# PNP-team/ZPrize23-gpu-submission

Hardware: AMD Instinct MI355X
Metric: gen_proof wall-clock (s), HEIGHT=15 Poseidon tree, 1/2/4/8 MI355X + HBM GB/s (lower is better)
Workload: dtype u64

## Files before the change

### zprize23-gpu-submission_amd/csrc/fr29.cuh

```cuda
#pragma once
#include "field.cuh"
#include "fr29_consts.inc"

namespace pnp {

struct R29 {
    uint32_t l[9];
};

#define R29_M 0x1FFFFFFFu

__device__ __forceinline__ R29 r29_from_words(const uint32_t *v) {
    R29 r;
#pragma unroll
    for (int j = 0; j < 9; j++) {
        const int bit = 29 * j, w = bit >> 5, sh = bit & 31;
        uint32_t x = v[w] >> sh;
        if (sh > 3 && w + 1 < 8) x |= v[w + 1] << (32 - sh);
        r.l[j] = j < 8 ? (x & R29_M) : x;
    }
    return r;
}

__device__ __forceinline__ void r29_to_words(const R29 &a, uint32_t *v) {
// ... 60 lines not shown
    R29 r;
    uint64_t acc = 0;
#pragma unroll
    for (int k = 0; k < 17; k++) {
#pragma unroll
        for (int i = (k > 8 ? k - 8 : 0); i <= (k < 8 ? k : 8); i++) {
            acc += (uint64_t)a.l[i] * b.l[k - i];
            acc += (uint64_t)c.l[i] * d.l[k - i];
        }
#pragma unroll
        for (int i = (k > 8 ? k - 8 : 0); i < (k < 9 ? k : 9); i++) acc += (uint64_t)m[i] * R29_P[k - i];
        if (k < 9) {
            m[k] = (0u - (uint32_t)acc) & R29_M;
            acc += m[k];
        } else {
            r.l[k - 9] = (uint32_t)acc & R29_M;
        }
        acc >>= 29;
    }
    r.l[8] = (uint32_t)acc;
    return r;
}

__device__ __forceinline__ R29 r29_canon(const R29 &x) {
    const uint32_t q = (uint32_t)(((uint64_t)x.l[8] * R29_MU) >> 32);
    R29 y;
    uint64_t acc = 0;
#pragma unroll
    for (int i = 0; i < 8; i++) {
        acc += x.l[i] + (uint64_t)q * R29_C[i];
        y.l[i] = (uint32_t)acc & R29_M;
        acc >>= 29;
    }
    y.l[8] = (uint32_t)(acc + x.l[8] + (uint64_t)q * R29_C[8] - ((uint64_t)q << 29));
#pragma unroll
    for (int rep = 0; rep < 2; rep++) {
        R29 z;
        uint32_t c = 0;
#pragma unroll
        for (int i = 0; i < 8; i++) {
            const uint32_t t = y.l[i] + R29_C[i] + c;
            z.l[i] = t & R29_M;
            c = t >> 29;
        }
        const uint32_t t = y.l[8] + R29_C[8] + c;
        const bool ge = t >= (1u << 29);
// ... 17 lines not shown
```

### zprize23-gpu-submission_amd/csrc/protocol.h

```cpp
#pragma once
#include "pnp_internal.h"

namespace pnp {

__host__ __device__ inline Fr from_u64_limbs_dev(const uint64_t *l) {
    Fr r;
#pragma unroll
    for (int i = 0; i < 4; i++) {
        r.v[2 * i] = (uint32_t)l[i];
        r.v[2 * i + 1] = (uint32_t)(l[i] >> 32);
    }
    return r;
}

struct PermArgs {
    const uint64_t *w[4];
    const uint64_t *sigma[4];
    Fr bk[4];
    Fr beta, gamma, omega;
    const uint64_t *tw;
};

struct QuotArgs {
    const uint64_t *w8[4], *z8, *pi8, *f8, *t8, *h18, *h28, *z28, *l18;
    const uint64_t *q_m, *q_l, *q_r, *q_o, *q_4, *q_c, *q_hl, *q_hr, *q_h4, *q_arith, *q_lookup;
    const uint64_t *sig[4], *lin, *vh_inv;
    const uint64_t *l1v, *pinv;
    Fr c_pi;
    uint64_t n;
    uint32_t lg_n;
    Fr alpha, alpha2, beta, gamma, delta, eps, zeta, lsep;
    Fr bk[4], opd, eopd, sep2, sep3;
};

struct Quot29Args {
    const uint64_t *w8[4], *z8, *pi8;
    const uint64_t *q_m, *q_l, *q_r, *q_o, *q_4, *q_c, *q_hl, *q_hr, *q_h4, *q_arith;
    const uint64_t *sig[4], *lin;
    const uint64_t *vh_inv, *l1v, *pinv;
    uint32_t c_pi[9], alpha[9], alpha2[9], beta[9], gamma[9], one[9];
    uint64_t n;
    uint32_t lg_n;
};
void fr_to_r29_limbs(const Fr &a, uint32_t l[9]);
void k_quotient29(const Quot29Args &q, uint64_t N8, uint64_t *out, hipStream_t s);
void k_to_form29(const uint64_t *in, uint64_t *out, uint64_t n, hipStream_t s);

struct WidgetArgs {
    const uint64_t *w8[4], *q_l, *q_r, *q_c, *vh_inv;
    const uint64_t *sel[4];
    Fr sep[4];
    uint64_t n;
    uint32_t lg_n;
};

constexpr int LIN_MAX = 32;
struct LinArgs {
    int k;
    const uint64_t *p[LIN_MAX];
    Fr s[LIN_MAX];
};

void k_compress4(uint64_t *out, const uint64_t *t0, const uint64_t *t1, const uint64_t *t2,
                 const uint64_t *t3, const Fr &z, uint64_t n, hipStream_t s);
void k_query_f(uint64_t *out, const uint64_t *ql, uint64_t n_gates, const uint64_t *const w[4],
               const uint64_t *tc, const Fr &z, uint64_t n, hipStream_t s);
void k_perm_numden(uint64_t *num, uint64_t *den, const PermArgs &a, uint64_t n, hipStream_t s);
void k_lookup_nd(uint64_t *num, uint64_t *den, const uint64_t *f, const uint64_t *t,
                 const uint64_t *h1, const uint64_t *h2, const Fr &delta, const Fr &eps, uint64_t n,
                 hipStream_t s);
void k_mul_inplace(uint64_t *a, const uint64_t *b, uint64_t n, hipStream_t s);
bool k_any_nonzero(const uint64_t *v, uint64_t words, DevBuf &scratch, hipStream_t s);
void k_any_nonzero_n(const uint64_t *v, uint64_t words, uint64_t stride, int cnt, bool *nz, DevBuf &scratch,
                     hipStream_t s);
bool k_any_diff(const uint64_t *a, const uint64_t *b, uint64_t words, DevBuf &scratch, hipStream_t s);
void k_hash_words(const uint64_t *a, uint64_t words, DevBuf &scratch, hipStream_t s, uint64_t out[2]);
bool k_pack_affine(const uint8_t *src, uint64_t n, uint64_t stride, uint64_t x_off, uint64_t y_off,
                   uint64_t inf_off, uint64_t *dst, DevBuf &scratch, hipStream_t s);
void k_affine(uint64_t *out, const uint64_t *in, const Fr &a, const Fr &b, uint64_t n, hipStream_t s);
void k_quotient(const QuotArgs &q, uint64_t N8, uint64_t *out, hipStream_t s);
void k_lincomb(const LinArgs &a, uint64_t n, uint64_t *out, hipStream_t s);
void k_widgets(const WidgetArgs &g, uint64_t N8, uint64_t *out, hipStream_t s);
bool combine_split(pnp_ctx *ctx, const uint64_t *t, const uint64_t *f, uint64_t n, uint64_t *h1,
                   uint64_t *h2, hipStream_t s);
void k_proof_marker(hipStream_t s);

}
```

### zprize23-gpu-submission_amd/csrc/protocol.hip

```cpp
#include "pnp_internal.h"
#include "protocol.h"
#include "widgets.cuh"
#include "fr29.cuh"
#include <vector>

namespace pnp {

static inline uint32_t nblk(uint64_t threads, uint32_t bs = 256) {
    return (uint32_t)((threads + bs - 1) / bs);
}

__global__ void k_compress4_(uint64_t *out, const uint64_t *t0, const uint64_t *t1,
                             const uint64_t *t2, const uint64_t *t3, Fr z, uint64_t n) {
    uint64_t i = blockIdx.x * (uint64_t)blockDim.x + threadIdx.x;
    if (i >= n) return;
    Fr acc = load_fr(t3, i);
    acc = acc * z + load_fr(t2, i);
    acc = acc * z + load_fr(t1, i);
    acc = acc * z + load_fr(t0, i);
    store_fr(out, i, acc);
}
void k_compress4(uint64_t *out, const uint64_t *t0, const uint64_t *t1, const uint64_t *t2,
                 const uint64_t *t3, const Fr &z, uint64_t n, hipStream_t s) {
    hipLaunchKernelGGL(k_compress4_, dim3(nblk(n)), dim3(256), 0, s, out, t0, t1, t2, t3, z, n);
    PNP_HIP(hipGetLastError());
}
// ... 59 lines not shown
    Fr eopd = eps * opd;
    const uint64_t nx = (i + 1) & (n - 1);
    Fr tn = load_fr(t, nx), h1n = load_fr(h1, nx);
    Fr fi = load_fr(f, i), ti = load_fr(t, i), h1i = load_fr(h1, i), h2i = load_fr(h2, i);
    Fr r = (eopd + ti + delta * tn) * (opd * (eps + fi));
    Fr d = (h2i * delta + (eopd + h1i)) * ((eopd + h2i) + h1n * delta);
    store_fr(num, i, r);
    store_fr(den, i, d);
}
void k_lookup_nd(uint64_t *num, uint64_t *den, const uint64_t *f, const uint64_t *t,
                 const uint64_t *h1, const uint64_t *h2, const Fr &delta, const Fr &eps, uint64_t n,
                 hipStream_t s) {
    hipLaunchKernelGGL(k_lookup_nd_, dim3(nblk(n)), dim3(256), 0, s, num, den, f, t, h1, h2, delta, eps,
                       n);
    PNP_HIP(hipGetLastError());
}

__global__ void k_mul_inplace_(uint64_t *a, const uint64_t *b, uint64_t n) {
    uint64_t i = blockIdx.x * (uint64_t)blockDim.x + threadIdx.x;
    if (i < n) store_fr(a, i, load_fr(a, i) * load_fr(b, i));
}
void k_mul_inplace(uint64_t *a, const uint64_t *b, uint64_t n, hipStream_t s) {
    hipLaunchKernelGGL(k_mul_inplace_, dim3(nblk(n)), dim3(256), 0, s, a, b, n);
    PNP_HIP(hipGetLastError());
}

__global__ __launch_bounds__(256) void k_any_nonzero_(const uint64_t *v, uint64_t words, uint64_t stride,
                                                      unsigned *flag) {
    const ulonglong2 *p = reinterpret_cast<const ulonglong2 *>(v + stride * blockIdx.y);
    const uint64_t pairs = words / 2;
    uint64_t acc = 0;
    for (uint64_t i = blockIdx.x * (uint64_t)blockDim.x + threadIdx.x; i < pairs;
         i += (uint64_t)gridDim.x * blockDim.x) {
        const ulonglong2 x = p[i];
        acc |= x.x | x.y;
    }
    if (blockIdx.x == 0 && threadIdx.x == 0 && (words & 1)) acc |= v[stride * blockIdx.y + words - 1];
    if (__any(acc != 0) && (threadIdx.x & 63) == 0) atomicOr(flag + blockIdx.y, 1u);
}
void k_any_nonzero_n(const uint64_t *v, uint64_t words, uint64_t stride, int cnt, bool *nz, DevBuf &scratch,
                     hipStream_t s) {
    scratch.reserve(4 * (size_t)cnt + 16);
    unsigned *flag = static_cast<unsigned *>(scratch.p);
    PNP_HIP(hipMemsetAsync(flag, 0, 4 * (size_t)cnt, s));
    if (words) {
        uint64_t blocks = (words / 2 + 255) / 256;
// ... 157 lines not shown
    }
    if (q.z28) {
        Fr tt = ld(q.t8, i), ttn = ld(q.t8, nx);
        Fr h1 = ld(q.h18, i), h1n = ld(q.h18, nx), h2 = ld(q.h28, i);
        Fr z2 = load_fr(q.z28, i), z2n = load_fr(q.z28, nx);
        Fr lk = z2 * q.opd * (f + q.eps) * (tt + q.eopd + ttn * q.delta) * q.sep2;
        lk -= z2n * (h1 + q.eopd + h2 * q.delta) * (h2 + q.eopd + h1n * q.delta) * q.sep2;
        l1t += (z2 - Fr::one()) * q.sep3;
        num += lk;
    }
    if (q.l1v) {
        Fr r = fr_mul2(num, load_fr(q.vh_inv, i), l1t, load_fr(q.l1v, i));
        if (q.pinv) r += q.c_pi * load_fr(q.pinv, i);
        store_fr(out, i, r);
    } else {
        store_fr(out, i, (num + l1t * load_fr(q.l18, i)) * load_fr(q.vh_inv, i));
    }
}
void k_quotient(const QuotArgs &q, uint64_t N8, uint64_t *out, hipStream_t s) {
    hipLaunchKernelGGL(k_quotient_, dim3(nblk(N8)), dim3(256), 0, s, q, N8, out);
    PNP_HIP(hipGetLastError());
}

__device__ __forceinline__ R29 ld29(const uint64_t *p, uint64_t i) {
    const uint4 *q = reinterpret_cast<const uint4 *>(p + 4 * i);
    const uint4 lo = q[0], hi = q[1];
    const uint32_t w[8] = {lo.x, lo.y, lo.z, lo.w, hi.x, hi.y, hi.z, hi.w};
    return r29_from_words(w);
}
__device__ __forceinline__ R29 c29(const uint32_t *c) {
    R29 r;
#pragma unroll
    for (int k = 0; k < 9; k++) r.l[k] = c[k];
    return r;
}
__device__ __forceinline__ R29 pow5_29(const R29 &a) {
    const R29 a2 = r29_mul(a, a);
    return r29_mul(r29_mul(a2, a2), a);
}
__device__ __forceinline__ R29 add3_29(const R29 &a, const R29 &b, const R29 &c) {
    return r29_add(r29_add(a, b), c);
}

__global__ __launch_bounds__(256, 4) void k_quotient29_(Quot29Args q, uint64_t N8, uint64_t *out) {
    const uint64_t i = blockIdx.x * (uint64_t)blockDim.x + threadIdx.x;
    if (i >= N8) return;
    const uint64_t nx = next_in_block(i, q.n, q.lg_n);
    const R29 a = ld29(q.w8[0], i), b = ld29(q.w8[1], i), c = ld29(q.w8[2], i), d = ld29(q.w8[3], i);
    R29 acc = r29_mul2(a, ld29(q.q_l, i), b, ld29(q.q_r, i));
    if (q.q_m) acc = r29_add(acc, r29_mul(r29_mul(a, b), ld29(q.q_m, i)));
    acc = r29_add(acc, r29_mul2(c, ld29(q.q_o, i), d, ld29(q.q_4, i)));
    acc = r29_add(acc, r29_mul2(pow5_29(a), ld29(q.q_hl, i), pow5_29(b), ld29(q.q_hr, i)));
    acc = r29_add(acc, r29_mul(pow5_29(d), ld29(q.q_h4, i)));
    acc = r29_add(acc, ld29(q.q_c, i));
    R29 num = r29_mul(acc, ld29(q.q_arith, i));
    if (q.pi8) num = r29_add(num, ld29(q.pi8, i));
    const R29 beta = c29(q.beta), gamma = c29(q.gamma);
    const R29 xb = r29_mul(ld29(q.lin, i), beta);
    const R29 x2 = r29_add(xb, xb), x4 = r29_add(x2, x2), x8 = r29_add(x4, x4);
    const R29 xb7 = r29_sub(x8, xb, R29_KDIF[0]);
    const R29 xb13 = add3_29(x8, x4, xb), xb17 = add3_29(x8, x8, xb);
    R29 pa = r29_mul(add3_29(xb, a, gamma), add3_29(xb7, b, gamma));
    pa = r29_mul(pa, add3_29(xb13, c, gamma));
    pa = r29_mul(pa, add3_29(xb17, d, gamma));
    R29 pb = r29_mul(add3_29(r29_mul(ld29(q.sig[0], i), beta), a, gamma),
                     add3_29(r29_mul(ld29(q.sig[1], i), beta), b, gamma));
    pb = r29_mul(pb, add3_29(r29_mul(ld29(q.sig[2], i), beta), c, gamma));
    pb = r29_mul(pb, add3_29(r29_mul(ld29(q.sig[3], i), beta), d, gamma));
    const R29 zi = ld29(q.z8, i), zn = ld29(q.z8, nx);
    R29 zero;
#pragma unroll
    for (int k = 0; k < 9; k++) zero.l[k] = 0;
    const R29 nzn = r29_sub(zero, zn, R29_KDIF[0]);
    num = r29_add(num, r29_mul(r29_mul2(pa, zi, pb, nzn), c29(q.alpha)));
    const R29 l1t = r29_mul(r29_sub(zi, c29(q.one), R29_KDIF[0]), c29(q.alpha2));
    R29 r = r29_mul2(num, ld29(q.vh_inv, i), l1t, ld29(q.l1v, i));
    if (q.pinv) r = r29_add(r, r29_mul(c29(q.c_pi), ld29(q.pinv, i)));
    r = r29_canon(r);
    uint32_t w[8];
    r29_to_words(r, w);
    uint4 *o = reinterpret_cast<uint4 *>(out + 4 * i);
    o[0] = make_uint4(w[0], w[1], w[2], w[3]);
    o[1] = make_uint4(w[4], w[5], w[6], w[7]);
}
void k_quotient29(const Quot29Args &q, uint64_t N8, uint64_t *out, hipStream_t s) {
    hipLaunchKernelGGL(k_quotient29_, dim3(nblk(N8)), dim3(256), 0, s, q, N8, out);
    PNP_HIP(hipGetLastError());
}

__global__ void k_to_form29_(const uint64_t *in, uint64_t *out, uint64_t n) {
    const uint64_t i = blockIdx.x * (uint64_t)blockDim.x + threadIdx.x;
    if (i >= n) return;
    Fr x = load_fr(in, i);
#pragma unroll
    for (int k = 0; k < 5; k++) x = x + x;
    store_fr(out, i, x);
}
void k_to_form29(const uint64_t *in, uint64_t *out, uint64_t n, hipStream_t s) {
    hipLaunchKernelGGL(k_to_form29_, dim3(nblk(n)), dim3(256), 0, s, in, out, n);
    PNP_HIP(hipGetLastError());
}

void fr_to_r29_limbs(const Fr &a, uint32_t l[9]) {
    Fr x = a;
    for (int k = 0; k < 5; k++) x = x + x;
    for (int j = 0; j < 9; j++) {
        const int bit = 29 * j, w = bit >> 5, sh = bit & 31;
        uint64_t v = x.v[w] >> sh;
        if (w + 1 < 8) v |= (uint64_t)x.v[w + 1] << (32 - sh);
        l[j] = j < 8 ? (uint32_t)(v & 0x1FFFFFFFu) : (uint32_t)v;
    }
}

__global__ __launch_bounds__(256) void k_widgets_(WidgetArgs g, uint64_t N8, uint64_t *out) {
    uint64_t i = blockIdx.x * (uint64_t)blockDim.x + threadIdx.x;
    if (i >= N8) return;
    const uint64_t nx = next_in_block(i, g.n, g.lg_n);
    WidgetVals w;
    w.a = load_fr(g.w8[0], i);
    w.b = load_fr(g.w8[1], i);
    w.c = load_fr(g.w8[2], i);
    w.d = load_fr(g.w8[3], i);
    w.a_next = load_fr(g.w8[0], nx);
    w.b_next = load_fr(g.w8[1], nx);
    w.d_next = load_fr(g.w8[3], nx);
    w.q_l = load_fr(g.q_l, i);
    w.q_r = load_fr(g.q_r, i);
    w.q_c = load_fr(g.q_c, i);
    Fr acc = Fr::zero();
    if (g.sel[0]) acc += load_fr(g.sel[0], i) * w_range(g.sep[0], w);
    if (g.sel[1]) acc += load_fr(g.sel[1], i) * w_logic(g.sep[1], w);
    if (g.sel[2]) acc += load_fr(g.sel[2], i) * w_fbsm(g.sep[2], w);
    if (g.sel[3]) acc += load_fr(g.sel[3], i) * w_cadd(g.sep[3], w);
    store_fr(out, i, load_fr(out, i) + acc * load_fr(g.vh_inv, i));
// ... 30 lines not shown
```

### zprize23-gpu-submission_amd/csrc/prover.cpp

```cpp
#include <chrono>
#include <string.h>
#include "context.h"
#include "protocol.h"
#include "transcript.h"
#include "widgets.cuh"
#include <algorithm>
#include <stddef.h>

namespace pnp {

Fr fr_from_u64(uint64_t x) {
    Fr r = Fr::zero();
    r.v[0] = (uint32_t)x;
    r.v[1] = (uint32_t)(x >> 32);
    return to_mont(r);
}

Fr root_of_unity(uint32_t lg) {
    const uint64_t root32[4] = {13381757501831005802ULL, 6564924994866501612ULL,
                                789602057691799140ULL, 6625830629041353339ULL};
    return pow_u64(from_u64_limbs<FrP>(root32), 1ULL << (32 - lg));
}

namespace {
// ... 509 lines not shown
    if (!table_zero) q.t8 = lde_to("t8", table_poly, false);
    if (!h_zero) {
        q.h18 = lde_to("h18", h1_poly, false);
        q.h28 = lde_to("h28", h2_poly, false);
    }
    if (!closed) {
        uint64_t *l1 = ctx->buf("l1", n);
        k_geometric(l1, n, n_inv, Fr::one(), s);
        q.l18 = lde_to("l18", l1, false);
    }
    auto kb = [&](int r) { return key.key_block(KeyPoly(r)); };
    q.q_m = kb(kQm), q.q_l = kb(kQl), q.q_r = kb(kQr), q.q_o = kb(kQo), q.q_4 = kb(kQ4), q.q_c = kb(kQc);
    q.q_hl = kb(kQhl), q.q_hr = kb(kQhr), q.q_h4 = kb(kQh4), q.q_arith = kb(kQarith), q.q_lookup = kb(kQlookup);
    for (int j = 0; j < 4; j++) q.sig[j] = kb(kSig0 + j);
    q.lin = kb(kLin);
    q.vh_inv = kb(kVhInv);
    q.n = n, q.lg_n = lg;
    q.alpha = alpha, q.alpha2 = alpha2, q.beta = beta, q.gamma = gamma, q.delta = delta, q.eps = eps;
    q.zeta = zeta, q.lsep = lsep, q.opd = opd, q.eopd = eopd, q.sep2 = sep2, q.sep3 = sep3;
    for (int j = 0; j < 4; j++) q.bk[j] = bk[j];
    return q;
}

Quot29Args quotient29_args(const QuotArgs &q) {
    Quot29Args q2;
    for (int j = 0; j < 4; j++) q2.w8[j] = q.w8[j];
    q2.z8 = q.z8;
    q2.pi8 = q.pi8;
    q2.q_m = q.q_m, q2.q_l = q.q_l, q2.q_r = q.q_r, q2.q_o = q.q_o, q2.q_4 = q.q_4, q2.q_c = q.q_c;
    q2.q_hl = q.q_hl, q2.q_hr = q.q_hr, q2.q_h4 = q.q_h4, q2.q_arith = q.q_arith;
    for (int j = 0; j < 4; j++) q2.sig[j] = q.sig[j];
    q2.lin = q.lin;
    q2.vh_inv = q.vh_inv;
    q2.l1v = q.l1v;
    q2.pinv = q.pinv;
    fr_to_r29_limbs(q.pinv ? q.c_pi : Fr::zero(), q2.c_pi);
    fr_to_r29_limbs(q.alpha, q2.alpha);
    fr_to_r29_limbs(q.alpha2, q2.alpha2);
    fr_to_r29_limbs(q.beta, q2.beta);
    fr_to_r29_limbs(q.gamma, q2.gamma);
    fr_to_r29_limbs(Fr::one(), q2.one);
    q2.n = q.n;
    q2.lg_n = q.lg_n;
    if (!q2.l1v || !q2.q_l || !q2.lin || !q2.sig[3]) fail(PNP_E_ARG, "quotient29: key copies missing");
    return q2;
}

void Proof::quotient_launch(const QuotArgs &q, int nbq, uint64_t *t_blk) {
    const uint64_t NBq = (uint64_t)nbq * n;
    hipEvent_t qe0 = nullptr;
    ctx->ktimer.begin("quotient", s, qe0);
    if (q29) {
        k_quotient29(quotient29_args(q), NBq, t_blk, s);
        ctx->ktimer.credit("quotient_points", (double)NBq);
        ctx->ktimer.credit("quotient_fr_products", (double)NBq * (34 + (q.q_m ? 2 : 0) + (q.pinv ? 1 : 0)));
    } else {
        k_quotient(q, NBq, t_blk, s);
    }
    if (ctx->key.any_custom()) {
        WidgetArgs g;
        for (int j = 0; j < 4; j++) g.w8[j] = q.w8[j];
        g.q_l = q.q_l, g.q_r = q.q_r, g.q_c = q.q_c, g.vh_inv = q.vh_inv;
        for (int k = 0; k < 4; k++) g.sel[k] = ctx->key.key_block(KeyPoly(kRange + k));
        g.sep[0] = range_c, g.sep[1] = logic_c, g.sep[2] = fixed_c, g.sep[3] = var_c;
        g.n = n, g.lg_n = lg;
        k_widgets(g, NBq, t_blk, s);
    }
    const uint64_t *arrs[] = {q.w8[0], q.w8[1], q.w8[2], q.w8[3], q.q_m, q.q_l, q.q_r, q.q_o,
                              q.q_4, q.q_c, q.q_hl, q.q_hr, q.q_h4, q.q_arith, q.pi8, q.lin,
                              q.z8, q.sig[0], q.sig[1], q.sig[2], q.sig[3], q.f8,
                              q.t8, q.h18, q.h28, q.q_lookup, q.z28, q.l18, q.vh_inv, q.l1v, q.pinv};
    int nread = 0;
    for (const uint64_t *a : arrs) nread += a != nullptr;
    ctx->ktimer.end("quotient", s, qe0, 32.0 * (double)NBq * (nread + 1));
    alg((double)NBq * (nread + 1));
}

const unsigned *Proof::quotient_chunks(int nbq, uint64_t *t_blk) {
    const uint64_t NBq = (uint64_t)nbq * n;
    intt_blocks(ctx->ntt, t_blk, lg, mb0, nbq, s);
    alg(2.0 * NBq + 2.0 * NBq);
    t_poly = ctx->buf("t_poly", 8 * len);
    unsigned *t_nz = reinterpret_cast<unsigned *>(ctx->buf("t_nz", 1));
    PNP_HIP(hipMemsetAsync(t_nz, 0, 4, s));
    if (!dist) {
        t_combine_blocks(ctx->ntt, t_blk, nbq, t_poly, lg, t_nz, s);
        return t_nz;
    }
    const uint64_t slot = (uint64_t)nb * len * 32;
    if (!ctx->msm.alltoall || ctx->msm.a2a_bytes < 2 * slot * world)
        fail(PNP_E_ARG, "round-4 all-to-all buffer missing or < %llu B", (unsigned long long)(2 * slot * world));
    uint64_t *a2a = ctx->msm.a2a;
    for (int r = 0; r < world; r++) {
        uint64_t r0, r1;
        msm_point_range(n, r, world, r0, r1);
// ... 283 lines not shown
```

### zprize23-gpu-submission_amd/csrc/prover_key.cpp

```cpp
#include <algorithm>
#include <chrono>
#include <string.h>
#include "context.h"
#include "ec.cuh"
#include "protocol.h"

using namespace pnp;

namespace {

bool host_all_zero(const uint64_t *p, uint64_t words) {
    uint64_t acc = 0;
    for (uint64_t i = 0; i < words; i++) acc |= p[i];
    return acc == 0;
}


void pk_begin_load(pnp_ctx *ctx) {
    tables_wait(ctx);
    PNP_HIP(hipSetDevice(ctx->device));
    ctx->key.loaded = false;
    ctx->key.wire_map_drop();
    ctx->key.gen++;
}
// ... 40 lines not shown
bool pk_q29_class(pnp_ctx *ctx, const ProverKeyC &dev, uint64_t D) {
    static const bool q29_on = [] {
        const char *e = getenv("PNP_QUOT29");
        return !e || atoi(e) != 0;
    }();
    const ResidentKey &key = ctx->key;
    bool q29 = q29_on && key.std_coset && key.qlookup_zero() && !key.any_custom();
    const uint64_t *const *f = reinterpret_cast<const uint64_t *const *>(&dev);
    for (int t = kTable1; t <= kTable4 && q29; t++) {
        const uint64_t *tab = f[kKeyTable[t].coeffs];
        q29 = !tab || !k_any_nonzero(tab, 4 * D, ctx->scratch_b, ctx->stream);
    }
    return q29;
}
void pk_sigma_domain(pnp_ctx *ctx, const ProverKeyC &dev, uint64_t D, uint32_t lg) {
    const uint64_t *const *f = reinterpret_cast<const uint64_t *const *>(&dev);
    for (int j = 0; j < 4; j++) {
        DevBuf &sn = ctx->key.sigma_n[j];
        sn.reserve(32 * D);
        PNP_HIP(hipMemcpyAsync(sn.p, f[kKeyTable[kSig0 + j].coeffs], 32 * D, hipMemcpyDeviceToDevice, ctx->stream));
        ntt_run(ctx->ntt, sn.u64(), lg, false, false, ctx->stream);
    }
}
template <class Make>
void pk_build_blocks(pnp_ctx *ctx, uint64_t D, bool q29, Make make) {
    ResidentKey &key = ctx->key;
    const size_t bytes = 32 * (size_t)key.nb * D;
    bool filled[kKeyRows] = {}, filled29[kKeyRows] = {};
    auto slot = [&](DevBuf &b) {
        if (b.bytes != bytes) b.alloc(bytes);
        return b.u64();
    };
    for (const KeyRow &r : kKeyTable) {
        if (r.cls == kTable || !key.has(r.id) || (r.id == kL1v && !key.std_coset)) continue;
        filled29[r.id] = q29 && r.in29;
        filled[r.id] = !filled29[r.id] || r.keeps256;
        uint64_t *d256 = filled[r.id] ? slot(key.blk[r.id]) : nullptr;
        uint64_t *d29 = filled29[r.id] ? slot(key.blk29[r.id]) : nullptr;
        make(r, d256, d29);
    }
    for (int r = 0; r < kKeyRows; r++) {
        if (!filled[r]) key.blk[r].release();
        if (!filled29[r]) key.blk29[r].release();
    }
    key.q29 = q29;
}
void pk_load_done(pnp_ctx *ctx, const ProverKeyC &dev, uint64_t D) {
    ResidentKey &key = ctx->key;
    key.blk_rank = ctx->msm.rank;
    key.blk_world = ctx->msm.world;
    key.pinv.release();
    key.pinv_pos = ~0ULL;
    PNP_HIP(hipStreamSynchronize(ctx->stream));
    key.dev = dev;
    key.n = D;
    key.loaded = true;
    ctx->hbm_checked = false;
}

void pk_derive_from_coeffs(pnp_ctx *ctx, ProverKeyC &dev, uint64_t D) {
    ResidentKey &key = ctx->key;
    uint64_t **dst = reinterpret_cast<uint64_t **>(&dev);
    for (int f = 0; f < kPkFields; f++) {
// ... 368 lines not shown
```

### zprize23-gpu-submission_amd/csrc/prover_key.h

```cpp
#pragma once
#include "pnp_internal.h"
#include <stddef.h>

namespace pnp {

enum KeyPoly : int {
    kQm, kQlookup, kRange, kLogic, kFixedAdd, kVarAdd,
    kQl, kQr, kQo, kQ4, kQc, kQhl, kQhr, kQh4, kQarith,
    kSig0, kSig1, kSig2, kSig3,
    kTable1, kTable2, kTable3, kTable4,
    kLin, kVhInv, kL1v,
    kKeyRows
};
enum KeyClass : int { kSel, kOptSel, kSigma, kTable, kCoset };
constexpr int kPkFields = 44;

struct KeyRow {
    KeyPoly id;
    const char *name;
    int coeffs, evals;
    KeyClass cls;
    bool in29, keeps256;
    int desc;
    int vk;
// ... 8 lines not shown
    {kFixedAdd, "fixed_add", 24, 25, kOptSel, false, false, 12, 12},
    {kVarAdd, "var_add", 26, 27, kOptSel, false, false, 13, 13},
    {kQl, "q_l", 2, 3, kSel, true, false, 1, 1},
    {kQr, "q_r", 4, 5, kSel, true, false, 2, 2},
    {kQo, "q_o", 6, 7, kSel, true, false, 3, 3},
    {kQ4, "q_4", 8, 9, kSel, true, false, 4, 4},
    {kQc, "q_c", 10, 11, kSel, true, false, 5, 5},
    {kQhl, "q_hl", 12, 13, kSel, true, false, 6, 6},
    {kQhr, "q_hr", 14, 15, kSel, true, false, 7, 7},
    {kQh4, "q_h4", 16, 17, kSel, true, false, 8, 8},
    {kQarith, "q_arith", 18, 19, kSel, true, false, 9, 9},
    {kSig0, "sig0", 34, 35, kSigma, true, false, -1, 14},
    {kSig1, "sig1", 36, 37, kSigma, true, false, -1, 15},
    {kSig2, "sig2", 38, 39, kSigma, true, false, -1, 16},
    {kSig3, "sig3", 40, 41, kSigma, true, false, -1, 17},
    {kTable1, "table1", 30, -1, kTable, false, false, -1, 19},
    {kTable2, "table2", 31, -1, kTable, false, false, -1, 20},
    {kTable3, "table3", 32, -1, kTable, false, false, -1, 21},
    {kTable4, "table4", 33, -1, kTable, false, false, -1, 22},
    {kLin, "lin", -1, 42, kCoset, true, true, -1, -1},
    {kVhInv, "vh_inv", -1, 43, kCoset, false, false, -1, -1},
    {kL1v, "l1v", -1, -1, kCoset, false, false, -1, -1},
};

#define PNP_KEY_ROW(r, co, ev)                                                                        \
    static_assert(kKeyTable[r].id == r, "kKeyTable is indexed by KeyPoly");                           \
    static_assert(offsetof(ProverKeyC, co) == 8 * kKeyTable[r].coeffs, "ProverKeyC." #co);           \
    static_assert(offsetof(ProverKeyC, ev) == 8 * kKeyTable[r].evals, "ProverKeyC." #ev)
#define PNP_KEY_ROW1(r, member, f)                                                                    \
    static_assert(kKeyTable[r].id == r, "kKeyTable is indexed by KeyPoly");                           \
    static_assert(offsetof(ProverKeyC, f) == 8 * kKeyTable[r].member, "ProverKeyC." #f)
PNP_KEY_ROW(kQm, q_m_coeffs, q_m_evals);
PNP_KEY_ROW(kQlookup, q_lookup_coeffs, q_lookup_evals);
PNP_KEY_ROW(kRange, range_selector_coeffs, range_selector_evals);
PNP_KEY_ROW(kLogic, logic_selector_coeffs, logic_selector_evals);
PNP_KEY_ROW(kFixedAdd, fixed_group_add_selector_coeffs, fixed_group_add_selector_evals);
PNP_KEY_ROW(kVarAdd, variable_group_add_selector_coeffs, variable_group_add_selector_evals);
PNP_KEY_ROW(kQl, q_l_coeffs, q_l_evals);
PNP_KEY_ROW(kQr, q_r_coeffs, q_r_evals);
PNP_KEY_ROW(kQo, q_o_coeffs, q_o_evals);
PNP_KEY_ROW(kQ4, q_4_coeffs, q_4_evals);
PNP_KEY_ROW(kQc, q_c_coeffs, q_c_evals);
PNP_KEY_ROW(kQhl, q_hl_coeffs, q_hl_evals);
PNP_KEY_ROW(kQhr, q_hr_coeffs, q_hr_evals);
PNP_KEY_ROW(kQh4, q_h4_coeffs, q_h4_evals);
PNP_KEY_ROW(kQarith, q_arith_coeffs, q_arith_evals);
// ... 39 lines not shown
}

struct ResidentKey {
    bool loaded = false;
    uint64_t n = 0;
    DevBuf owned[kPkFields];
    ProverKeyC dev{};
    uint64_t gen = 0;
    uint32_t present = 0;
    bool has(KeyPoly r) const { return !kKeyTable[r].optional() || (present >> r & 1); }
    bool qm_zero() const { return !has(kQm); }
    bool qlookup_zero() const { return !has(kQlookup); }
    bool custom(int k) const { return has(KeyPoly(kRange + k)); }
    bool any_custom() const { return custom(0) || custom(1) || custom(2) || custom(3); }
    void set_present(const ProverKeyC &d) {
        const uint64_t *const *f = reinterpret_cast<const uint64_t *const *>(&d);
        present = 0;
        for (const KeyRow &r : kKeyTable)
            if (r.optional() && (f[r.coeffs] || f[r.evals])) present |= 1u << r.id;
    }
    DevBuf sigma_n[4];
    DevBuf tmp[4];
    DevBuf blk[kKeyRows], blk29[kKeyRows];
    int mb0 = 0, nb = 8, blk_rank = 0, blk_world = 1;
    bool std_coset = false, q29 = false;
    const uint64_t *key_block(KeyPoly r) const { return (q29 && kKeyTable[r].in29 ? blk29[r] : blk[r]).u64(); }
    DevBuf pinv;
    uint64_t pinv_pos = ~0ULL;

    bool wm_loaded = false;
    uint64_t wm_gates = 0, wm_vars = 0;
    DevBuf wm_var;
    DevBuf wm_qlk;
    void wire_map_drop() {
        wm_loaded = false;
        wm_gates = wm_vars = 0;
        wm_var.release();
        wm_qlk.release();
        solve.drop();
    }

    struct SolvePlan {
        bool loaded = false;
        uint64_t n_inputs = 0, n_solved = 0, n_levels = 0;
        DevBuf buf;
        SolveView view{};
// ... 19 lines not shown
```

### zprize23-gpu-submission_amd/csrc/v1.cpp

```cpp
#include <algorithm>
#include <array>
#include <atomic>
#include <chrono>
#include <thread>
#include <stdlib.h>
#include <string.h>
#include "context.h"
#include "protocol.h"

using namespace pnp;

namespace {

using clk = std::chrono::steady_clock;
double ms_since(clk::time_point a) { return std::chrono::duration<double, std::milli>(clk::now() - a).count(); }

struct ScopedThread {
    std::thread t;
    void join() {
        if (t.joinable()) t.join();
    }
    ~ScopedThread() { join(); }
};

// ... 136 lines not shown
struct V1KeyLoad {
    bool derive = false;
    bool tried = false, derived = false, fell_back = false;
    double ms_scan = 0, ms_derive = 0, ms_fallback = 0;
};
bool v1_sampled_check(pnp_ctx *ctx, const ProverKeyC &pk, uint64_t D) {
    uint64_t *const *f = reinterpret_cast<uint64_t *const *>(&pk);
    const uint64_t K = 256, words = 4 * 8 * D;
    const uint32_t lg = log2_exact(D);
    std::vector<uint64_t> idx(K + 1);
    for (uint64_t k = 0; k <= K; k++) idx[k] = ((words - 1) * k / K) / 4;
    const uint32_t cnt = (uint32_t)idx.size();
    struct Arr {
        int field;
        int form;
    };
    std::vector<Arr> arrs;
    std::vector<const uint64_t *> blks;
    for (int i = 0; i < kPkFields; i++) {
        const KeyField fld = key_field(i);
        if (!fld.evals) continue;
        if (!f[i]) return false;
        const uint64_t *b = ctx->key.blk[fld.row->id].u64(), *b29 = ctx->key.blk29[fld.row->id].u64();
        arrs.push_back({i, fld.row->id == kVhInv ? 3 : b ? 1 : b29 ? 2 : 0});
        blks.push_back(b ? b : b29);
    }
    pnp::DevBuf d_idx(8 * cnt), d_out(32 * (size_t)cnt * arrs.size());
    std::vector<uint64_t> got(4 * (size_t)cnt * arrs.size());
    PNP_HIP(hipMemcpyAsync(d_idx.p, idx.data(), 8 * cnt, hipMemcpyHostToDevice, ctx->stream));
    for (size_t a = 0; a < arrs.size(); a++)
        if (blks[a])
            pnp::k_gather_blocks(blks[a], lg, ctx->key.mb0, ctx->key.nb, d_idx.u64(), cnt, d_out.u64() + 4 * cnt * a,
                                 ctx->stream);
    PNP_HIP(hipMemcpyAsync(got.data(), d_out.p, 8 * got.size(), hipMemcpyDeviceToHost, ctx->stream));
    PNP_HIP(hipStreamSynchronize(ctx->stream));
    const uint64_t zero[4] = {0, 0, 0, 0};
    uint64_t one[4];
    to_u64_limbs(Fr::one(), one);
    for (size_t a = 0; a < arrs.size(); a++) {
        const uint64_t *src = f[arrs[a].field];
        for (uint32_t k = 0; k < cnt; k++) {
            const int m = (int)(idx[k] & 7);
            const uint64_t *mine = src + 4 * idx[k], *dev = &got[4 * (cnt * a + k)];
            if (arrs[a].form == 0) {
                if (memcmp(mine, zero, 32)) return false;
                continue;
            }
            if (m < ctx->key.mb0 || m >= ctx->key.mb0 + ctx->key.nb) continue;
            uint64_t want[4];
            if (arrs[a].form == 1) {
                memcpy(want, mine, 32);
            } else if (arrs[a].form == 2) {
                Fr x = from_u64_limbs<FrP>(mine);
                for (int d = 0; d < 5; d++) x = x + x;
                to_u64_limbs(x, want);
            } else {
                to_u64_limbs(from_u64_limbs<FrP>(mine) * from_u64_limbs<FrP>(dev), want);
                dev = one;
            }
            if (memcmp(want, dev, 32)) return false;
        }
    }
    return true;
}
int v1_load_prover_key(pnp_ctx *ctx, const ProverKeyC &pk, uint64_t D, V1KeyLoad &st, unsigned cap = 0) {
    if (!st.derive) return pnp_load_prover_key(ctx, &pk, D, 0);
    st.tried = true;
    uint64_t *const *f = reinterpret_cast<uint64_t *const *>(&pk);
    bool usable = true;
    for (const KeyRow &r : kKeyTable)
        if (r.optional()) usable &= f[r.evals] != nullptr;
    if (usable) {
        auto t = clk::now();
        std::vector<Seg> segs;
        std::vector<int> coeffs;
        for (const KeyRow &r : kKeyTable)
            if (r.optional()) {
                segs.push_back({f[r.evals], 4 * D});
// ... 253 lines not shown
```

Baseline: 0.1182.

## Restructure quotient29 with premultiplied selectors, beta-normalized permutation, and fused products

Selector key blocks (q_m, q_l..q_h4) are premultiplied once at key load by q_arith and the per-coset-block constant vh_inv, so the kernel no longer reads q_arith or vh_inv arrays. The permutation terms are divided through by beta, so sigma and lin no longer need a beta multiply, and beta^4·alpha·vh_inv is folded into a per-block constant. Gate terms are factored as w*(q_lin + w^4*q_h) and computed with a new squaring routine and 3- and 4-way fused Montgomery products, which cuts the multiply and reduction count per point. It also checks that vh_inv is constant per block and falls back to the old path otherwise. This adds key-load work and more complex validation logic.

```diff
diff --git a/zprize23-gpu-submission_amd/csrc/fr29.cuh b/zprize23-gpu-submission_amd/csrc/fr29.cuh
--- a/zprize23-gpu-submission_amd/csrc/fr29.cuh
+++ b/zprize23-gpu-submission_amd/csrc/fr29.cuh
@@ -106,6 +106,86 @@
     return r;
 }
 
+__device__ __forceinline__ R29 r29_sqr(const R29 &a) {
+    uint32_t m[9], a2[9];
+    R29 r;
+    uint64_t acc = 0;
+#pragma unroll
+    for (int i = 0; i < 9; i++) a2[i] = a.l[i] << 1;
+#pragma unroll
+    for (int k = 0; k < 17; k++) {
+#pragma unroll
+        for (int i = (k > 8 ? k - 8 : 0); 2 * i < k; i++) acc += (uint64_t)a2[i] * a.l[k - i];
+        if (!(k & 1)) acc += (uint64_t)a.l[k >> 1] * a.l[k >> 1];
+#pragma unroll
+        for (int i = (k > 8 ? k - 8 : 0); i < (k < 9 ? k : 9); i++) acc += (uint64_t)m[i] * R29_P[k - i];
+        if (k < 9) {
+            m[k] = (0u - (uint32_t)acc) & R29_M;
+            acc += m[k];
+        } else {
+            r.l[k - 9] = (uint32_t)acc & R29_M;
+        }
+        acc >>= 29;
+    }
+    r.l[8] = (uint32_t)acc;
+    return r;
+}
+
+__device__ __forceinline__ R29 r29_mul3(const R29 &a, const R29 &b, const R29 &c, const R29 &d, const R29 &e,
+                                        const R29 &f) {
+    uint32_t m[9];
+    R29 r;
+    uint64_t acc = 0;
+#pragma unroll
+    for (int k = 0; k < 17; k++) {
+#pragma unroll
+        for (int i = (k > 8 ? k - 8 : 0); i <= (k < 8 ? k : 8); i++) {
+            acc += (uint64_t)a.l[i] * b.l[k - i];
+            acc += (uint64_t)c.l[i] * d.l[k - i];
+            acc += (uint64_t)e.l[i] * f.l[k - i];
+        }
+#pragma unroll
+        for (int i = (k > 8 ? k - 8 : 0); i < (k < 9 ? k : 9); i++) acc += (uint64_t)m[i] * R29_P[k - i];
+        if (k < 9) {
+            m[k] = (0u - (uint32_t)acc) & R29_M;
+            acc += m[k];
+        } else {
+            r.l[k - 9] = (uint32_t)acc & R29_M;
+        }
+        acc >>= 29;
+    }
+    r.l[8] = (uint32_t)acc;
+    return r;
+}
+
+__device__ __forceinline__ R29 r29_mul4(const R29 &a, const R29 &b, const R29 &c, const R29 &d, const R29 &e,
+                                        const R29 &f, const R29 &g, const R29 &h) {
+    uint32_t m[9];
+    R29 r;
+    uint64_t acc = 0;
+#pragma unroll
+    for (int k = 0; k < 17; k++) {
+#pragma unroll
+        for (int i = (k > 8 ? k - 8 : 0); i <= (k < 8 ? k : 8); i++) {
+            acc += (uint64_t)a.l[i] * b.l[k - i];
+            acc += (uint64_t)c.l[i] * d.l[k - i];
+            acc += (uint64_t)e.l[i] * f.l[k - i];
+            acc += (uint64_t)g.l[i] * h.l[k - i];
+        }
+#pragma unroll
+        for (int i = (k > 8 ? k - 8 : 0); i < (k < 9 ? k : 9); i++) acc += (uint64_t)m[i] * R29_P[k - i];
+        if (k < 9) {
+            m[k] = (0u - (uint32_t)acc) & R29_M;
+            acc += m[k];
+        } else {
+            r.l[k - 9] = (uint32_t)acc & R29_M;
+        }
+        acc >>= 29;
+    }
+    r.l[8] = (uint32_t)acc;
+    return r;
+}
+
 __device__ __forceinline__ R29 r29_canon(const R29 &x) {
     const uint32_t q = (uint32_t)(((uint64_t)x.l[8] * R29_MU) >> 32);
     R29 y;
diff --git a/zprize23-gpu-submission_amd/csrc/protocol.h b/zprize23-gpu-submission_amd/csrc/protocol.h
--- a/zprize23-gpu-submission_amd/csrc/protocol.h
+++ b/zprize23-gpu-submission_amd/csrc/protocol.h
@@ -35,13 +35,16 @@
 
 struct Quot29Args {
     const uint64_t *w8[4], *z8, *pi8;
-    const uint64_t *q_m, *q_l, *q_r, *q_o, *q_4, *q_c, *q_hl, *q_hr, *q_h4, *q_arith;
+    const uint64_t *q_m, *q_l, *q_r, *q_o, *q_4, *q_c, *q_hl, *q_hr, *q_h4;
     const uint64_t *sig[4], *lin;
-    const uint64_t *vh_inv, *l1v, *pinv;
-    uint32_t c_pi[9], alpha[9], alpha2[9], beta[9], gamma[9], one[9];
+    const uint64_t *l1v, *pinv;
+    uint32_t km[8][9], vhm[8][9];
+    uint32_t c_pi[9], alpha2[9], binv[9], gamma[9], one[9];
+    uint32_t beta0;
     uint64_t n;
     uint32_t lg_n;
 };
+void fr_to_r29_words(const Fr &a, uint32_t l[9]);
 void fr_to_r29_limbs(const Fr &a, uint32_t l[9]);
 void k_quotient29(const Quot29Args &q, uint64_t N8, uint64_t *out, hipStream_t s);
 void k_to_form29(const uint64_t *in, uint64_t *out, uint64_t n, hipStream_t s);
@@ -70,6 +73,7 @@
                  const uint64_t *h1, const uint64_t *h2, const Fr &delta, const Fr &eps, uint64_t n,
                  hipStream_t s);
 void k_mul_inplace(uint64_t *a, const uint64_t *b, uint64_t n, hipStream_t s);
+void k_mul_const_inplace(uint64_t *a, const uint64_t *b, const Fr &c, uint64_t n, hipStream_t s);
 bool k_any_nonzero(const uint64_t *v, uint64_t words, DevBuf &scratch, hipStream_t s);
 void k_any_nonzero_n(const uint64_t *v, uint64_t words, uint64_t stride, int cnt, bool *nz, DevBuf &scratch,
                      hipStream_t s);
diff --git a/zprize23-gpu-submission_amd/csrc/protocol.hip b/zprize23-gpu-submission_amd/csrc/protocol.hip
--- a/zprize23-gpu-submission_amd/csrc/protocol.hip
+++ b/zprize23-gpu-submission_amd/csrc/protocol.hip
@@ -1,7 +1,7 @@
 #include "pnp_internal.h"
 #include "protocol.h"
 #include "widgets.cuh"
-#include "fr29.cuh"
+#include "quot29.cuh"
 #include <vector>
 
 namespace pnp {
@@ -107,6 +107,15 @@
 }
 void k_mul_inplace(uint64_t *a, const uint64_t *b, uint64_t n, hipStream_t s) {
     hipLaunchKernelGGL(k_mul_inplace_, dim3(nblk(n)), dim3(256), 0, s, a, b, n);
+    PNP_HIP(hipGetLastError());
+}
+
+__global__ void k_mul_const_inplace_(uint64_t *a, const uint64_t *b, Fr c, uint64_t n) {
+    uint64_t i = blockIdx.x * (uint64_t)blockDim.x + threadIdx.x;
+    if (i < n) store_fr(a, i, load_fr(a, i) * load_fr(b, i) * c);
+}
+void k_mul_const_inplace(uint64_t *a, const uint64_t *b, const Fr &c, uint64_t n, hipStream_t s) {
+    hipLaunchKernelGGL(k_mul_const_inplace_, dim3(nblk(n)), dim3(256), 0, s, a, b, c, n);
     PNP_HIP(hipGetLastError());
 }
 
@@ -310,61 +319,10 @@
     PNP_HIP(hipGetLastError());
 }
 
-__device__ __forceinline__ R29 ld29(const uint64_t *p, uint64_t i) {
-    const uint4 *q = reinterpret_cast<const uint4 *>(p + 4 * i);
-    const uint4 lo = q[0], hi = q[1];
-    const uint32_t w[8] = {lo.x, lo.y, lo.z, lo.w, hi.x, hi.y, hi.z, hi.w};
-    return r29_from_words(w);
-}
-__device__ __forceinline__ R29 c29(const uint32_t *c) {
-    R29 r;
-#pragma unroll
-    for (int k = 0; k < 9; k++) r.l[k] = c[k];
-    return r;
-}
-__device__ __forceinline__ R29 pow5_29(const R29 &a) {
-    const R29 a2 = r29_mul(a, a);
-    return r29_mul(r29_mul(a2, a2), a);
-}
-__device__ __forceinline__ R29 add3_29(const R29 &a, const R29 &b, const R29 &c) {
-    return r29_add(r29_add(a, b), c);
-}
-
 __global__ __launch_bounds__(256, 4) void k_quotient29_(Quot29Args q, uint64_t N8, uint64_t *out) {
     const uint64_t i = blockIdx.x * (uint64_t)blockDim.x + threadIdx.x;
     if (i >= N8) return;
-    const uint64_t nx = next_in_block(i, q.n, q.lg_n);
-    const R29 a = ld29(q.w8[0], i), b = ld29(q.w8[1], i), c = ld29(q.w8[2], i), d = ld29(q.w8[3], i);
-    R29 acc = r29_mul2(a, ld29(q.q_l, i), b, ld29(q.q_r, i));
-    if (q.q_m) acc = r29_add(acc, r29_mul(r29_mul(a, b), ld29(q.q_m, i)));
-    acc = r29_add(acc, r29_mul2(c, ld29(q.q_o, i), d, ld29(q.q_4, i)));
-    acc = r29_add(acc, r29_mul2(pow5_29(a), ld29(q.q_hl, i), pow5_29(b), ld29(q.q_hr, i)));
-    acc = r29_add(acc, r29_mul(pow5_29(d), ld29(q.q_h4, i)));
-    acc = r29_add(acc, ld29(q.q_c, i));
-    R29 num = r29_mul(acc, ld29(q.q_arith, i));
-    if (q.pi8) num = r29_add(num, ld29(q.pi8, i));
-    const R29 beta = c29(q.beta), gamma = c29(q.gamma);
-    const R29 xb = r29_mul(ld29(q.lin, i), beta);
-    const R29 x2 = r29_add(xb, xb), x4 = r29_add(x2, x2), x8 = r29_add(x4, x4);
-    const R29 xb7 = r29_sub(x8, xb, R29_KDIF[0]);
-    const R29 xb13 = add3_29(x8, x4, xb), xb17 = add3_29(x8, x8, xb);
-    R29 pa = r29_mul(add3_29(xb, a, gamma), add3_29(xb7, b, gamma));
-    pa = r29_mul(pa, add3_29(xb13, c, gamma));
-    pa = r29_mul(pa, add3_29(xb17, d, gamma));
-    R29 pb = r29_mul(add3_29(r29_mul(ld29(q.sig[0], i), beta), a, gamma),
-                     add3_29(r29_mul(ld29(q.sig[1], i), beta), b, gamma));
-    pb = r29_mul(pb, add3_29(r29_mul(ld29(q.sig[2], i), beta), c, gamma));
-    pb = r29_mul(pb, add3_29(r29_mul(ld29(q.sig[3], i), beta), d, gamma));
-    const R29 zi = ld29(q.z8, i), zn = ld29(q.z8, nx);
-    R29 zero;
-#pragma unroll
-    for (int k = 0; k < 9; k++) zero.l[k] = 0;
-    const R29 nzn = r29_sub(zero, zn, R29_KDIF[0]);
-    num = r29_add(num, r29_mul(r29_mul2(pa, zi, pb, nzn), c29(q.alpha)));
-    const R29 l1t = r29_mul(r29_sub(zi, c29(q.one), R29_KDIF[0]), c29(q.alpha2));
-    R29 r = r29_mul2(num, ld29(q.vh_inv, i), l1t, ld29(q.l1v, i));
-    if (q.pinv) r = r29_add(r, r29_mul(c29(q.c_pi), ld29(q.pinv, i)));
-    r = r29_canon(r);
+    const R29 r = quot29_point(q, i, next_in_block(i, q.n, q.lg_n), (uint32_t)(i >> q.lg_n));
     uint32_t w[8];
     r29_to_words(r, w);
     uint4 *o = reinterpret_cast<uint4 *>(out + 4 * i);
@@ -389,15 +347,18 @@
     PNP_HIP(hipGetLastError());
 }
 
-void fr_to_r29_limbs(const Fr &a, uint32_t l[9]) {
-    Fr x = a;
-    for (int k = 0; k < 5; k++) x = x + x;
+void fr_to_r29_words(const Fr &x, uint32_t l[9]) {
     for (int j = 0; j < 9; j++) {
         const int bit = 29 * j, w = bit >> 5, sh = bit & 31;
         uint64_t v = x.v[w] >> sh;
         if (w + 1 < 8) v |= (uint64_t)x.v[w + 1] << (32 - sh);
         l[j] = j < 8 ? (uint32_t)(v & 0x1FFFFFFFu) : (uint32_t)v;
     }
+}
+void fr_to_r29_limbs(const Fr &a, uint32_t l[9]) {
+    Fr x = a;
+    for (int k = 0; k < 5; k++) x = x + x;
+    fr_to_r29_words(x, l);
 }
 
 __global__ __launch_bounds__(256) void k_widgets_(WidgetArgs g, uint64_t N8, uint64_t *out) {
diff --git a/zprize23-gpu-submission_amd/csrc/prover.cpp b/zprize23-gpu-submission_amd/csrc/prover.cpp
--- a/zprize23-gpu-submission_amd/csrc/prover.cpp
+++ b/zprize23-gpu-submission_amd/csrc/prover.cpp
@@ -555,22 +555,27 @@
     return q;
 }
 
-Quot29Args quotient29_args(const QuotArgs &q) {
-    Quot29Args q2;
+Quot29Args quotient29_args(const QuotArgs &q, const Fr *vh_inv_m, int mb0, int nb) {
+    Quot29Args q2{};
     for (int j = 0; j < 4; j++) q2.w8[j] = q.w8[j];
     q2.z8 = q.z8;
     q2.pi8 = q.pi8;
     q2.q_m = q.q_m, q2.q_l = q.q_l, q2.q_r = q.q_r, q2.q_o = q.q_o, q2.q_4 = q.q_4, q2.q_c = q.q_c;
-    q2.q_hl = q.q_hl, q2.q_hr = q.q_hr, q2.q_h4 = q.q_h4, q2.q_arith = q.q_arith;
+    q2.q_hl = q.q_hl, q2.q_hr = q.q_hr, q2.q_h4 = q.q_h4;
     for (int j = 0; j < 4; j++) q2.sig[j] = q.sig[j];
     q2.lin = q.lin;
-    q2.vh_inv = q.vh_inv;
     q2.l1v = q.l1v;
     q2.pinv = q.pinv;
+    q2.beta0 = q.beta == Fr::zero();
+    const Fr b2 = q.beta * q.beta;
+    const Fr ab4 = q2.beta0 ? q.alpha : q.alpha * b2 * b2;
+    for (int k = 0; k < nb; k++) {
+        fr_to_r29_words(ab4 * vh_inv_m[mb0 + k], q2.km[k]);
+        fr_to_r29_words(vh_inv_m[mb0 + k], q2.vhm[k]);
+    }
     fr_to_r29_limbs(q.pinv ? q.c_pi : Fr::zero(), q2.c_pi);
-    fr_to_r29_limbs(q.alpha, q2.alpha);
     fr_to_r29_limbs(q.alpha2, q2.alpha2);
-    fr_to_r29_limbs(q.beta, q2.beta);
+    fr_to_r29_limbs(q2.beta0 ? Fr::one() : inverse(q.beta), q2.binv);
     fr_to_r29_limbs(q.gamma, q2.gamma);
     fr_to_r29_limbs(Fr::one(), q2.one);
     q2.n = q.n;
@@ -584,9 +589,10 @@
     hipEvent_t qe0 = nullptr;
     ctx->ktimer.begin("quotient", s, qe0);
     if (q29) {
-        k_quotient29(quotient29_args(q), NBq, t_blk, s);
+        k_quotient29(quotient29_args(q, ctx->key.vh_inv_m, mb0, nbq), NBq, t_blk, s);
         ctx->ktimer.credit("quotient_points", (double)NBq);
-        ctx->ktimer.credit("quotient_fr_products", (double)NBq * (34 + (q.q_m ? 2 : 0) + (q.pinv ? 1 : 0)));
+        ctx->ktimer.credit("quotient_fr_products",
+                           (double)NBq * (28 + (q.q_m ? 2 : 0) + (q.pinv || q.pi8 ? 1 : 0)));
     } else {
         k_quotient(q, NBq, t_blk, s);
     }
@@ -600,10 +606,10 @@
         k_widgets(g, NBq, t_blk, s);
     }
     const uint64_t *arrs[] = {q.w8[0], q.w8[1], q.w8[2], q.w8[3], q.q_m, q.q_l, q.q_r, q.q_o,
-                              q.q_4, q.q_c, q.q_hl, q.q_hr, q.q_h4, q.q_arith, q.pi8, q.lin,
+                              q.q_4, q.q_c, q.q_hl, q.q_hr, q.q_h4, q.pi8, q.lin,
                               q.z8, q.sig[0], q.sig[1], q.sig[2], q.sig[3], q.f8,
-                              q.t8, q.h18, q.h28, q.q_lookup, q.z28, q.l18, q.vh_inv, q.l1v, q.pinv};
-    int nread = 0;
+                              q.t8, q.h18, q.h28, q.q_lookup, q.z28, q.l18, q.l1v, q.pinv};
+    int nread = q29 ? 0 : 2;
     for (const uint64_t *a : arrs) nread += a != nullptr;
     ctx->ktimer.end("quotient", s, qe0, 32.0 * (double)NBq * (nread + 1));
     alg((double)NBq * (nread + 1));
diff --git a/zprize23-gpu-submission_amd/csrc/prover_key.cpp b/zprize23-gpu-submission_amd/csrc/prover_key.cpp
--- a/zprize23-gpu-submission_amd/csrc/prover_key.cpp
+++ b/zprize23-gpu-submission_amd/csrc/prover_key.cpp
@@ -86,6 +86,33 @@
         ntt_run(ctx->ntt, sn.u64(), lg, false, false, ctx->stream);
     }
 }
+bool pk_vh_block_consts(pnp_ctx *ctx, uint64_t D) {
+    ResidentKey &key = ctx->key;
+    const uint64_t *v = key.blk[kVhInv].u64();
+    uint64_t h[8][4];
+    for (int k = 0; k < key.nb; k++) {
+        const uint64_t *b = v + 4 * (uint64_t)k * D;
+        if (k_any_diff(b + 4, b, 4 * (D - 1), ctx->scratch_b, ctx->stream)) return false;
+        PNP_HIP(hipMemcpyAsync(h[k], b, 32, hipMemcpyDeviceToHost, ctx->stream));
+    }
+    PNP_HIP(hipStreamSynchronize(ctx->stream));
+    for (int k = 0; k < key.nb; k++) key.vh_inv_m[key.mb0 + k] = from_u64_limbs<FrP>(h[k]);
+    return true;
+}
+void pk_premultiply(pnp_ctx *ctx, uint64_t D) {
+    ResidentKey &key = ctx->key;
+    Fr k1024 = Fr::zero();
+    k1024.v[0] = 1024;
+    const Fr c = inverse(to_mont(k1024));
+    for (const KeyRow &r : kKeyTable) {
+        if (!key_row_premultiplied(r.id) || !key.blk29[r.id].u64()) continue;
+        for (int k = 0; k < key.nb; k++) {
+            const uint64_t off = 4 * (uint64_t)k * D;
+            k_mul_const_inplace(key.blk29[r.id].u64() + off, key.blk29[kQarith].u64() + off,
+                                key.vh_inv_m[key.mb0 + k] * c, D, ctx->stream);
+        }
+    }
+}
 template <class Make>
 void pk_build_blocks(pnp_ctx *ctx, uint64_t D, bool q29, Make make) {
     ResidentKey &key = ctx->key;
@@ -95,14 +122,24 @@
         if (b.bytes != bytes) b.alloc(bytes);
         return b.u64();
     };
-    for (const KeyRow &r : kKeyTable) {
-        if (r.cls == kTable || !key.has(r.id) || (r.id == kL1v && !key.std_coset)) continue;
-        filled29[r.id] = q29 && r.in29;
-        filled[r.id] = !filled29[r.id] || r.keeps256;
-        uint64_t *d256 = filled[r.id] ? slot(key.blk[r.id]) : nullptr;
-        uint64_t *d29 = filled29[r.id] ? slot(key.blk29[r.id]) : nullptr;
-        make(r, d256, d29);
-    }
+    auto walk = [&](bool coset) {
+        for (const KeyRow &r : kKeyTable) {
+            if ((r.cls == kCoset) != coset) continue;
+            if (r.cls == kTable || !key.has(r.id) || (r.id == kL1v && !key.std_coset)) continue;
+            filled29[r.id] = q29 && r.in29;
+            filled[r.id] = !filled29[r.id] || r.keeps256;
+            uint64_t *d256 = filled[r.id] ? slot(key.blk[r.id]) : nullptr;
+            uint64_t *d29 = filled29[r.id] ? slot(key.blk29[r.id]) : nullptr;
+            make(r, d256, d29);
+        }
+    };
+    walk(true);
+    if (q29 && !pk_vh_block_consts(ctx, D)) {
+        q29 = false;
+        filled29[kLin] = false;
+    }
+    walk(false);
+    if (q29) pk_premultiply(ctx, D);
     for (int r = 0; r < kKeyRows; r++) {
         if (!filled[r]) key.blk[r].release();
         if (!filled29[r]) key.blk29[r].release();
diff --git a/zprize23-gpu-submission_amd/csrc/prover_key.h b/zprize23-gpu-submission_amd/csrc/prover_key.h
--- a/zprize23-gpu-submission_amd/csrc/prover_key.h
+++ b/zprize23-gpu-submission_amd/csrc/prover_key.h
@@ -54,6 +54,8 @@
     {kVhInv, "vh_inv", -1, 43, kCoset, false, false, -1, -1},
     {kL1v, "l1v", -1, -1, kCoset, false, false, -1, -1},
 };
+
+constexpr bool key_row_premultiplied(KeyPoly r) { return r == kQm || (r >= kQl && r <= kQh4); }
 
 #define PNP_KEY_ROW(r, co, ev)                                                                        \
     static_assert(kKeyTable[r].id == r, "kKeyTable is indexed by KeyPoly");                           \
@@ -139,6 +141,7 @@
     DevBuf sigma_n[4];
     DevBuf tmp[4];
     DevBuf blk[kKeyRows], blk29[kKeyRows];
+    Fr vh_inv_m[8];
     int mb0 = 0, nb = 8, blk_rank = 0, blk_world = 1;
     bool std_coset = false, q29 = false;
     const uint64_t *key_block(KeyPoly r) const { return (q29 && kKeyTable[r].in29 ? blk29[r] : blk[r]).u64(); }
diff --git a/zprize23-gpu-submission_amd/csrc/quot29.cuh b/zprize23-gpu-submission_amd/csrc/quot29.cuh
--- /dev/null
+++ b/zprize23-gpu-submission_amd/csrc/quot29.cuh
@@ -0,0 +1,71 @@
+#pragma once
+#include "fr29.cuh"
+#include "protocol.h"
+
+namespace pnp {
+
+__device__ __forceinline__ R29 ld29(const uint64_t *p, uint64_t i) {
+    const uint4 *q = reinterpret_cast<const uint4 *>(p + 4 * i);
+    const uint4 lo = q[0], hi = q[1];
+    const uint32_t w[8] = {lo.x, lo.y, lo.z, lo.w, hi.x, hi.y, hi.z, hi.w};
+    return r29_from_words(w);
+}
+__device__ __forceinline__ R29 c29(const uint32_t *c) {
+    R29 r;
+#pragma unroll
+    for (int k = 0; k < 9; k++) r.l[k] = c[k];
+    return r;
+}
+__device__ __forceinline__ R29 add3_29(const R29 &a, const R29 &b, const R29 &c) {
+    return r29_add(r29_add(a, b), c);
+}
+__device__ __forceinline__ R29 gate_sel29(const R29 &w, const R29 &q_lin, const R29 &q_h) {
+    const R29 w2 = r29_sqr(w);
+    return r29_add(q_lin, r29_mul(r29_sqr(w2), q_h));
+}
+
+__device__ __forceinline__ R29 quot29_point(const Quot29Args &q, uint64_t i, uint64_t nx, uint32_t m) {
+    const R29 a = ld29(q.w8[0], i), b = ld29(q.w8[1], i), c = ld29(q.w8[2], i), d = ld29(q.w8[3], i);
+    R29 acc;
+    {
+        const R29 sa = gate_sel29(a, ld29(q.q_l, i), ld29(q.q_hl, i));
+        const R29 sb = gate_sel29(b, ld29(q.q_r, i), ld29(q.q_hr, i));
+        const R29 sd = gate_sel29(d, ld29(q.q_4, i), ld29(q.q_h4, i));
+        acc = r29_add(r29_mul4(a, sa, b, sb, d, sd, c, ld29(q.q_o, i)), ld29(q.q_c, i));
+    }
+    if (q.q_m) acc = r29_add(acc, r29_mul(r29_mul(a, b), ld29(q.q_m, i)));
+    const R29 binv = c29(q.binv), gamma = c29(q.gamma);
+    const R29 wa = r29_mul(r29_add(a, gamma), binv), wb = r29_mul(r29_add(b, gamma), binv);
+    const R29 wc = r29_mul(r29_add(c, gamma), binv), wd = r29_mul(r29_add(d, gamma), binv);
+    R29 zero;
+#pragma unroll
+    for (int k = 0; k < 9; k++) zero.l[k] = 0;
+    R29 pa, pb;
+    {
+        const R29 x = q.beta0 ? zero : ld29(q.lin, i);
+        const R29 x2 = r29_add(x, x), x4 = r29_add(x2, x2), x8 = r29_add(x4, x4);
+        const R29 x7 = r29_sub(x8, x, R29_KDIF[0]);
+        pa = r29_mul(r29_add(x, wa), r29_add(x7, wb));
+        pa = r29_mul(pa, r29_add(add3_29(x8, x4, x), wc));
+        pa = r29_mul(pa, r29_add(add3_29(x8, x8, x), wd));
+    }
+    if (q.beta0) {
+        pb = r29_mul(r29_mul(r29_mul(wa, wb), wc), wd);
+    } else {
+        pb = r29_mul(r29_add(ld29(q.sig[0], i), wa), r29_add(ld29(q.sig[1], i), wb));
+        pb = r29_mul(pb, r29_add(ld29(q.sig[2], i), wc));
+        pb = r29_mul(pb, r29_add(ld29(q.sig[3], i), wd));
+    }
+    const R29 zi = ld29(q.z8, i);
+    const R29 nzn = r29_sub(zero, ld29(q.z8, nx), R29_KDIF[0]);
+    const R29 perm = r29_mul2(pa, zi, pb, nzn);
+    const R29 l1t = r29_mul(r29_sub(zi, c29(q.one), R29_KDIF[0]), c29(q.alpha2));
+    const R29 km = c29(q.km[m]), l1v = ld29(q.l1v, i);
+    R29 r;
+    if (q.pinv) r = r29_mul3(perm, km, l1t, l1v, c29(q.c_pi), ld29(q.pinv, i));
+    else if (q.pi8) r = r29_mul3(perm, km, l1t, l1v, ld29(q.pi8, i), c29(q.vhm[m]));
+    else r = r29_mul2(perm, km, l1t, l1v);
+    return r29_canon(r29_add(acc, r));
+}
+
+}
diff --git a/zprize23-gpu-submission_amd/csrc/v1.cpp b/zprize23-gpu-submission_amd/csrc/v1.cpp
--- a/zprize23-gpu-submission_amd/csrc/v1.cpp
+++ b/zprize23-gpu-submission_amd/csrc/v1.cpp
@@ -182,7 +182,7 @@
         if (!fld.evals) continue;
         if (!f[i]) return false;
         const uint64_t *b = ctx->key.blk[fld.row->id].u64(), *b29 = ctx->key.blk29[fld.row->id].u64();
-        arrs.push_back({i, fld.row->id == kVhInv ? 3 : b ? 1 : b29 ? 2 : 0});
+        arrs.push_back({i, fld.row->id == kVhInv ? 3 : b ? 1 : !b29 ? 0 : key_row_premultiplied(fld.row->id) ? 4 : 2});
         blks.push_back(b ? b : b29);
     }
     pnp::DevBuf d_idx(8 * cnt), d_out(32 * (size_t)cnt * arrs.size());
@@ -197,6 +197,16 @@
     const uint64_t zero[4] = {0, 0, 0, 0};
     uint64_t one[4];
     to_u64_limbs(Fr::one(), one);
+    std::vector<Fr> premul;
+    auto premul_at = [&](uint32_t k) {
+        if (premul.empty()) {
+            premul.resize(cnt);
+            for (uint32_t j = 0; j < cnt; j++)
+                premul[j] = from_u64_limbs<FrP>(f[kKeyTable[kQarith].evals] + 4 * idx[j]) *
+                            inverse(from_u64_limbs<FrP>(f[kKeyTable[kVhInv].evals] + 4 * idx[j]));
+        }
+        return premul[k];
+    };
     for (size_t a = 0; a < arrs.size(); a++) {
         const uint64_t *src = f[arrs[a].field];
         for (uint32_t k = 0; k < cnt; k++) {
@@ -214,6 +224,8 @@
                 Fr x = from_u64_limbs<FrP>(mine);
                 for (int d = 0; d < 5; d++) x = x + x;
                 to_u64_limbs(x, want);
+            } else if (arrs[a].form == 4) {
+                to_u64_limbs(from_u64_limbs<FrP>(mine) * premul_at(k), want);
             } else {
                 to_u64_limbs(from_u64_limbs<FrP>(mine) * from_u64_limbs<FrP>(dev), want);
                 dev = one;
```

Measured after the change: 0.1171, median of 6. About the same (-1.0%).
